# Nazukixv/LiteASR

Hardware: AMD Instinct MI355X
Metric: utterances/sec (U2-Conformer+CTC, 80-d fbank T≈1000) at 1/2/4/8 MI355X (higher is better)
Workload: dtype bf16; 1 GPU; U2-Conformer-small hybrid CTC-attention training step (fwd+loss+bwd+allreduce+clip+Noam/Adam); model=U2 enc 12x conformer d256 H4 ff2048, dec 6x, V 4233, global_batch=32, per_gpu_batch=32, seq_len=1000, label_len=40, parallelism=dp1, launch=hipgraph, ranks_seen=1, rank_launcher=env

## Files before the change

### include/liteasr_hip.h

```cpp
#ifndef LITEASR_HIP_H
#define LITEASR_HIP_H

#include <stdint.h>

#ifdef __cplusplus
extern "C" {
#endif

enum { LASR_F32 = 0, LASR_BF16 = 1, LASR_I32 = 2, LASR_I64 = 3, LASR_U8 = 4 };
enum { LASR_OK = 0, LASR_ERR_INVALID = -1, LASR_ERR_LAUNCH = -2 };
enum { LASR_ACT_NONE = 0, LASR_ACT_RELU = 1, LASR_ACT_SWISH = 2,
       LASR_ACT_GATE = 3 ,
       LASR_ACT_TANH = 4  };

const char* lasr_last_error(void);
int lasr_version(void);
int lasr_set_dropout_counter(const uint64_t* dev_counter);
int lasr_counter_add(uint64_t* dev_counter, uint64_t v, void* stream);

typedef struct lasr_gemm_args {
  int M, N, K;
  int batch, batch_div;
  const void* A; int64_t lda_m, lda_k, sa1, sa2;
  const void* B; int64_t ldb_n, ldb_k, sb1, sb2;
// ... 13 lines not shown
  float* rowsum;
  int zout_mode;
  int tile_m, tile_n;
  int ksub;
} lasr_gemm_args;
int lasr_gemm(const lasr_gemm_args* args, void* stream);
int lasr_gemm_ln_fwd(const lasr_gemm_args* args, const float* gamma, const float* beta, float eps, void* y,
                     int y_dtype, float* mean, float* rstd, void* stream);
int lasr_gemm_ln_bwd(const lasr_gemm_args* args, const void* x, int x_dtype, const float* gamma, const float* mean,
                     const float* rstd, const void* dres, int dres_dtype, void* dx, int dx_dtype, float* part,
                     int64_t part_floats, void* gb, int gb_dtype, float bscale, float bp, uint64_t bseed,
                     void* stream);
int lasr_gemm_qbias_bwd(const lasr_gemm_args* args, const void* dqu, const void* dqv, int dt, int B, int T, int H,
                        int dk, void* dqkv, int64_t ld, float* ws, int64_t ws_floats, void* stream);
float lasr_dropout_scale(float p);
#define LASR_PLAN_GLDS 1
#define LASR_PLAN_ROWSUM_FUSED 2
#define LASR_PLAN_KSUB2 4
#define LASR_PLAN_WIDE 8
int lasr_gemm_plan(const lasr_gemm_args* args, int* tile_m, int* tile_n, int* split_k, int* flags);

int lasr_gemm_dw_group(const lasr_gemm_args* args, int n, void* stream);
int lasr_gemm_dw_group_order(int longest_first);
int lasr_gemm_narrow_tiles(int on);
int lasr_gemm_phased(int mode);
long long lasr_gemm_phased_launches(void);

typedef struct lasr_reduce_seg {
  const float* part; int64_t N; int P; int accumulate;
  float* out0; float* out1; int64_t split;
} lasr_reduce_seg;
int lasr_reduce_multi(const lasr_reduce_seg* segs, int nseg, void* stream);

int lasr_colsum(const void* X, int dtype, int64_t M, int64_t N, int64_t ldx,
                float* out, int accumulate, float* workspace, int64_t ws_floats, void* stream);

int lasr_layernorm_fwd(const void* x, int x_dtype, int64_t rows, int D, const float* gamma,
                       const float* beta, float eps, void* y, int y_dtype, float* mean,
                       float* rstd, void* y2, int y2_dtype, float p2, uint64_t seed2,
                       void* stream);
int lasr_layernorm2_fwd(const float* x, int64_t rows, int D, const float* g1, const float* b1,
                        const float* g2, const float* b2, float eps, float* y, float* mean1,
                        float* rstd1, void* z, float* mean2, float* rstd2, void* stream);
int lasr_layernorm_bwd(const void* x, int x_dtype, const void* dy, int dy_dtype, int64_t rows,
                       int D, const float* gamma, const float* mean, const float* rstd,
                       const void* dres, int dres_dtype, void* dx, int dx_dtype,
// ... 318 lines not shown
```

### liteasr_amd/_native.py

```python

from __future__ import annotations

import ctypes as C
import os

_HERE = os.path.dirname(os.path.abspath(__file__))
LIB_PATH = os.path.join(_HERE, "lib", "libliteasr_hip.so")

F32, BF16, I32, I64, U8 = 0, 1, 2, 3, 4
ACT_NONE, ACT_RELU, ACT_SWISH, ACT_GATE, ACT_TANH = 0, 1, 2, 3, 4

_p = C.c_void_p
_i = C.c_int
_l = C.c_int64
_f = C.c_float
_u = C.c_uint64


class GemmArgs(C.Structure):

    _fields_ = [
        ("M", _i), ("N", _i), ("K", _i),
        ("batch", _i), ("batch_div", _i),
        ("A", _p), ("lda_m", _l), ("lda_k", _l), ("sa1", _l), ("sa2", _l),
# ... 78 lines not shown
class RnntSearchArgs(C.Structure):

    _fields_ = [
        ("Tcap", _i), ("layers", _i), ("dec_dim", _i), ("H", _i), ("J", _i), ("V", _i),
        ("node_cap", _i), ("slot_cap", _i),
        ("w_dtype", _i),
        ("arena", _p), ("arena_bytes", _l),
        ("embed", _p),
        ("Wih", _p * RNNT_SEARCH_MAX_LAYERS), ("Whh", _p * RNNT_SEARCH_MAX_LAYERS),
        ("bih", _p * RNNT_SEARCH_MAX_LAYERS), ("bhh", _p * RNNT_SEARCH_MAX_LAYERS),
        ("Wd", _p), ("Wj", _p), ("bj", _p), ("enc_proj", _p),
    ]


SIGNATURES = {
    "lasr_version": [],
    "lasr_last_error": [],
    "lasr_set_dropout_counter": [_p],
    "lasr_counter_add": [_p, _u, _p],
    "lasr_gemm": [C.POINTER(GemmArgs), _p],
    "lasr_gemm_plan": [C.POINTER(GemmArgs), _p, _p, _p, _p],
    "lasr_gemm_dw_group": [C.POINTER(GemmArgs), _i, _p],
    "lasr_gemm_dw_group_order": [_i],
    "lasr_gemm_narrow_tiles": [_i],
    "lasr_gemm_phased": [_i],
    "lasr_gemm_phased_launches": [],
    "lasr_relattn_fwd": [_p, _p, _l, _p, _p, _l, _p, _l, _i, _i, _i, _i, _p, _l, _l, _f, _p, _p, _l, _p],
    "lasr_relattn_fwd_qb": [_p, _l, _p, _p, _p, _p, _l, _p, _p, _l, _p, _l, _i, _i, _i, _i, _p, _l, _l, _f, _p, _p,
                            _l, _p],
    "lasr_attn_fwd": [_p, _l, _p, _p, _l, _i, _i, _i, _i, _i, _p, _l, _l, _f, _p, _p, _l, _p],
    "lasr_attn_bwd": [_p, _l, _p, _p, _l, _i, _i, _i, _i, _i, _p, _l, _l, _f, _p, _p, _p, _l, _p, _p, _p, _p,
                      _l, _p],
    "lasr_attn_fwd_split": [_p, _l, _p, _p, _l, _i, _i, _i, _i, _i, _p, _l, _l, _f, _p, _p, _l, _i, _p, _l, _p],
    "lasr_attn_bwd_split": [_p, _l, _p, _p, _l, _i, _i, _i, _i, _i, _p, _l, _l, _f, _p, _p, _p, _l, _p, _p, _p,
                            _p, _l, _i, _p, _l, _p],
    "lasr_attn_split_work": [_i, _i, _i, _i, _i],
    "lasr_attn_split_count": [_i, _i, _i, _i],
    "lasr_relattn_bwd": [_p, _p, _l, _p, _p, _l, _p, _l, _i, _i, _i, _i, _p, _l, _l, _f, _p, _p, _p, _l,
                         _p, _p, _p, _i, _i, _p, _p, _l, _p],
    "lasr_reduce_multi": [C.POINTER(ReduceSeg), _i, _p],
    "lasr_linear_res_ln": [C.POINTER(RowLnArgs), _p],
    "lasr_linear_dx_ln_bwd": [C.POINTER(RowLnArgs), _p],
    "lasr_dropout_scale": [_f],
    "lasr_colsum": [_p, _i, _l, _l, _l, _p, _i, _p, _l, _p],
    "lasr_layernorm2_fwd": [_p, _l, _i, _p, _p, _p, _p, _f, _p, _p, _p, _p, _p, _p, _p],
    "lasr_layernorm_fwd": [_p, _i, _l, _i, _p, _p, _f, _p, _i, _p, _p, _p, _i, _f, _u, _p],
# ... 77 lines not shown
    "lasr_rescore_pick_batch": [_p, _l, _i, _i, _i, _p, C.c_double, _p],
    "lasr_w2v_conv0_fwd": [_p, _i, _i, _i, _i, _i, _p, _p, _p, _p],
    "lasr_w2v_conv0_dw_parts": [_i, _i],
    "lasr_w2v_conv0_dw": [_p, _p, _i, _i, _i, _i, _i, _i, _p, _p, _l, _p],
    "lasr_w2v_ln_act_fwd": [_p, _i, _l, _i, _p, _p, _f, _i, _p, _i, _p, _p, _p],
    "lasr_w2v_ln_act_bwd": [_p, _i, _p, _i, _l, _i, _p, _p, _p, _p, _i, _p, _i, _p, _p, _p, _l, _p],
    "lasr_w2v_col2im1d": [_p, _i, _i, _i, _i, _i, _i, _i, _p, _p],
    "lasr_w2v_group_pack": [_p, _i, _i, _i, _i, _i, _i, _p, _i, _p, _p, _i, _p],
    "lasr_w2v_group_unpack": [_p, _i, _p, _i, _p, _i, _i, _i, _i, _p, _p],
    "lasr_w2v_group_colsum": [_p, _i, _i, _l, _i, _p, _p],
    "lasr_w2v_mask_fwd": [_p, _p, _i, _i, _i, _i, _p, _p],
    "lasr_w2v_mask_bwd": [_p, _p, _i, _i, _i, _i, _p, _p],
    "lasr_w2v_gather_rows": [_p, _i, _l, _l, _p, _i, _i, _i, _i, _p, _i, _p],
    "lasr_w2v_scatter_rows": [_p, _i, _p, _i, _i, _i, _i, _p, _l, _l, _i, _p],
    "lasr_w2v_gumbel_fwd": [_p, _i, _p, _u, _f, _i, _l, _i, _i, _p, _i, _p, _i, _p, _p],
    "lasr_w2v_gumbel_bwd": [_p, _i, _p, _u, _f, _i, _l, _i, _i, _p, _i, _p, _i, _p, _p, _i, _p, _p],
    "lasr_w2v_contrast_fwd": [_p, _p, _p, _p, _i, _i, _i, _i, _i, _f, _p, _p, _p, _p, _p],
    "lasr_w2v_contrast_bwd": [_p, _p, _p, _p, _i, _i, _i, _i, _i, _f, _p, _p, _p, _p, _p, _l, _p],
}
_RESTYPES = {"lasr_last_error": C.c_char_p, "lasr_spec_augment_ws_bytes": C.c_int64,
             "lasr_rnnt_search_workspace": C.c_int64, "lasr_rescore_workspace": C.c_int64,
             "lasr_rescore_workspace_batch": C.c_int64, "lasr_ctc_align_workspace": C.c_int64,
             "lasr_conv2_dx_w1_workspace": C.c_int64, "lasr_attn_split_work": C.c_int64,
             "lasr_dropout_scale": C.c_float, "lasr_gemm_phased_launches": C.c_int64}


class NativeError(RuntimeError):
    pass


_lib = None


def load():
    global _lib
    if _lib is not None:
        return _lib
    want = os.environ.get("LITEASR_HIP_LIB")
    if want and os.path.abspath(want) != os.path.abspath(LIB_PATH):
        raise NativeError(f"LITEASR_HIP_LIB={want} does not select the library (this process loads {LIB_PATH}); "
                          "run `python tools/with_lib.py LIB script.py` to use another build")
    if not os.path.exists(LIB_PATH):
        raise NativeError(
            f"libliteasr_hip.so not found at {LIB_PATH}; build it with `make` "
            "(the HIP path has no fallback)"
        )
    lib = C.CDLL(LIB_PATH)
# ... 20 lines not shown
```

### liteasr_amd/csrc/gemm.hip

```cpp
#include "gemm_kernel.h"
#include "gemm_phase.h"
#include <algorithm>


template <bool AKC, bool BKC, typename TC>
void launch_bf16(const GemmP& p, int BM, int BN, int ks, int nw, bool glds, dim3 grid, hipStream_t st);
#define LASR_EXTERN_LAUNCH(ak, bk)                                                                         \
  extern template void launch_bf16<ak, bk, float>(const GemmP&, int, int, int, int, bool, dim3, hipStream_t); \
  extern template void launch_bf16<ak, bk, bf16_t>(const GemmP&, int, int, int, int, bool, dim3, hipStream_t);
LASR_EXTERN_LAUNCH(true, true)
LASR_EXTERN_LAUNCH(true, false)
LASR_EXTERN_LAUNCH(false, true)
LASR_EXTERN_LAUNCH(false, false)
#undef LASR_EXTERN_LAUNCH

template <typename TC>
static void dispatch(const GemmP& p, bool akc, bool bkc, int bf16in, int BM, int BN, int ks, int nw, bool glds,
                     dim3 grid, hipStream_t st) {
  if (bf16in) {
    if (akc && bkc) launch_bf16<true, true, TC>(p, BM, BN, ks, nw, glds, grid, st);
    else if (akc) launch_bf16<true, false, TC>(p, BM, BN, ks, nw, glds, grid, st);
    else if (bkc) launch_bf16<false, true, TC>(p, BM, BN, ks, nw, glds, grid, st);
    else launch_bf16<false, false, TC>(p, BM, BN, ks, nw, glds, grid, st);
  } else {
    if (akc && bkc) gemm_f32_kernel<true, true, TC><<<grid, 256, 0, st>>>(p);
// ... 204 lines not shown
    const int r = post->launch(p, post->ctx, st);
    if (r < 0) return r;
    post->done = r;
    if (r) {
      rc = lasr_check_launch("lasr_gemm/splitk_reduce_post");
      if (rc || !a->rowsum || rs_fused) return rc;
    }
  }
  if (!rc && split > 1 && a->split_k >= 0 && !(post && post->done)) {
    const int64_t total = (int64_t)a->M * a->N * batch;
    const int nblk = (int)std::min<int64_t>(cdiv(p.v4 ? total / 4 : total, 256), 4096);
    if (a->c_dtype == LASR_F32) splitk_reduce_kernel<float><<<nblk, 256, 0, st>>>(p);
    else splitk_reduce_kernel<bf16_t><<<nblk, 256, 0, st>>>(p);
    rc = lasr_check_launch("lasr_gemm/splitk_reduce");
  }
  if (rc || !a->rowsum || rs_fused) return rc;
  const int64_t used = split > 1 ? (int64_t)split * batch * a->M * a->N : 0;
  LASR_CHECK_ARG(a->workspace && a->workspace_bytes / 4 > used, "lasr_gemm: no workspace left for the rowsum");
  return lasr_colsum(a->A, a->in_dtype, a->K, a->M, a->lda_k, a->rowsum, 1, (float*)a->workspace + used,
                     a->workspace_bytes / 4 - used, stream);
}


int launch_dw_group(const DwGroupP& g, int BM, int BN, int blocks, bool serial, hipStream_t st);
static int dw_group_lpt = 1;
extern "C" int lasr_gemm_dw_group_order(int longest_first) {
  dw_group_lpt = longest_first != 0;
  return LASR_OK;
}

extern "C" int lasr_gemm_dw_group(const lasr_gemm_args* args, int n, void* stream) {
  LASR_CHECK_ARG(args && n >= 1 && n <= LASR_DW_GROUP_MAX, "lasr_gemm_dw_group: 1..%d problems", LASR_DW_GROUP_MAX);
  DwGroupP g = {};
  g.n = n;
  int ord[LASR_DW_GROUP_MAX];
  int64_t work[LASR_DW_GROUP_MAX];
  auto planned = [](const lasr_gemm_args* a) {
    lasr_gemm_args b = *a;
    if (b.split_k <= -2 && !b.workspace) {
      b.workspace = (void*)(uintptr_t)16;
      b.workspace_bytes = INT64_MAX;
    }
    return b;
  };
  for (int i = 0; i < n; ++i) {
    const lasr_gemm_args pa = planned(args + i), *a = &pa;
    int bm, bn, sp, ks;
    gemm_plan(a, &bm, &bn, &sp, &ks);
    work[i] = a->split_k == 1 || sp <= 1 ? a->K : cdiv(a->K, sp);
    ord[i] = i;
  }
  if (dw_group_lpt && !(args[0].split_k <= -2 && !args[0].workspace))
    std::stable_sort(ord, ord + n, [&](int x, int y) { return work[x] > work[y]; });
  int BM0 = 0, BN0 = 0, blocks = 0;
  bool all_serial = false;
  for (int i = 0; i < n; ++i) {
    const bool serial = args[ord[i]].split_k <= -2 && !args[ord[i]].workspace;
    const lasr_gemm_args pa = planned(args + ord[i]), *a = &pa;
    LASR_CHECK_ARG(a->in_dtype == LASR_BF16 && a->c_dtype == LASR_F32, "lasr_gemm_dw_group: bf16 in, fp32 partials");
    LASR_CHECK_ARG(a->lda_m == 1 && a->lda_k != 1 && a->ldb_n == 1 && a->ldb_k != 1,
                   "lasr_gemm_dw_group: A M-contiguous and B N-contiguous (dW = dY^T X)");
    const bool direct = a->split_k == 1;
    LASR_CHECK_ARG((direct || (a->split_k < 0 && a->workspace)) && (a->batch <= 1) && a->M > 0 && a->N > 0 &&
                       a->K > 0,
                   "lasr_gemm_dw_group: partials-only problems with a workspace, or direct (split_k 1) ones");
    LASR_CHECK_ARG(!serial || (a->C && a->ldc >= a->N && (a->beta == 0.f || a->beta == 1.f) && a->alpha == 1.f &&
                               !a->alpha_dev && a->split_k >= -64),
                   "lasr_gemm_dw_group: a serial problem needs C, ldc >= N, beta 0 or 1, alpha 1, <= 64 slices");
    LASR_CHECK_ARG(i == 0 || serial == all_serial, "lasr_gemm_dw_group: serial and slab problems mixed");
    all_serial = serial;
    LASR_CHECK_ARG(!direct || (a->C && a->ldc >= a->N && (a->beta == 0.f || a->beta == 1.f) && a->alpha == 1.f &&
                               !a->alpha_dev),
                   "lasr_gemm_dw_group: a direct problem needs C, ldc >= N, beta 0 or 1, alpha 1");
    LASR_CHECK_ARG(i == 0 || direct == (g.direct[0] != 0), "lasr_gemm_dw_group: direct and split problems mixed");
    LASR_CHECK_ARG(!a->act && !a->zout && !a->aux && !a->res && a->drop_p <= 0.f && !a->bias,
                   "lasr_gemm_dw_group: no epilogue");
    LASR_CHECK_ARG(gemm_uses_glds(a), "lasr_gemm_dw_group: operands not LDS-DMA eligible");
    int BM, BN, split, ks;
    gemm_plan(a, &BM, &BN, &split, &ks);
    if (direct) split = 2;
    LASR_CHECK_ARG(split > 1, "lasr_gemm_dw_group: plan is not a split-K launch");
    if (((BM == 128 && BN == 64) || (BM == 64 && BN == 128)) && a->M >= 128 && a->N >= 128) {
      BM = BN = 128;
      if (a->M >= 256 && a->N >= 256 && !direct) {
        BM = 256;
        BN = 128;
      }
    }
    LASR_CHECK_ARG(i == 0 || (BM == BM0 && BN == BN0), "lasr_gemm_dw_group: problems plan different tiles");
    BM0 = BM;
    BN0 = BN;
    if (direct) split = 1;
    g.M[i] = a->M; g.N[i] = a->N; g.K[i] = a->K;
    g.split[i] = split;
    g.kchunk[i] = direct ? a->K : (int)(cdiv(cdiv(a->K, split), 32) * 32);
    g.direct[i] = direct;
    g.C[i] = (float*)a->C; g.ldc[i] = a->ldc; g.beta[i] = a->beta; g.rowsum[i] = a->rowsum;
    g.v4[i] = serial ? a->N % 4 == 0 && aligned16(a->C) && a->ldc % 4 == 0
                     : a->N % 4 == 0 && aligned16(direct ? a->C : a->workspace);
    g.A[i] = a->A; g.lda[i] = a->lda_k;
    g.B[i] = a->B; g.ldb[i] = a->ldb_k;
    g.ws[i] = serial ? nullptr : (float*)a->workspace;
    g.rs_ws[i] = a->rowsum && !direct && !serial ? (float*)a->workspace + (int64_t)split * a->M * a->N : nullptr;
    g.start[i] = blocks;
    const int64_t nb = cdiv(a->M, BM) * cdiv(a->N, BN) * (int64_t)(serial ? 1 : split);
    LASR_CHECK_ARG(blocks + nb + 8 < (1ll << 31), "lasr_gemm_dw_group: too many blocks");
    blocks += (int)cdiv(nb, 8) * 8;
  }
  g.start[n] = blocks;
  static const int slice_xcd = [] { const char* e = getenv("LASR_DW_SLICE_XCD"); return e && e[0] ? atoi(e) : 1; }();
  g.slice_xcd = slice_xcd;
  LASR_CHECK_ARG(launch_dw_group(g, BM0, BN0, blocks, all_serial, (hipStream_t)stream) == 0,
                 "lasr_gemm_dw_group: no grouped instance for tile %dx%d", BM0, BN0);
  return lasr_check_launch("lasr_gemm_dw_group");
}
```

### liteasr_amd/csrc/gemm_group.hip

```cpp
#include "gemm_kernel.h"

static_assert(sizeof(DwGroupP) <= 4096, "DwGroupP must fit the kernel-argument block");

int launch_dw_group(const DwGroupP& g, int BM, int BN, int blocks, bool serial, hipStream_t st) {
  if (serial) {
    if (BM == 64 && BN == 64) gemm_dw_group_kernel<64, 64, 3, 3, 4, true><<<blocks, 256, 0, st>>>(g);
    else if (BM == 256 && BN == 128) gemm_dw_group_kernel<256, 128, 3, 1, 8, true><<<blocks, 512, 0, st>>>(g);
    else return -1;
    return 0;
  }
  if (BM == 64 && BN == 64) gemm_dw_group_kernel<64, 64, 3, 3><<<blocks, 256, 0, st>>>(g);
  else if (BM == 64 && BN == 128) gemm_dw_group_kernel<64, 128, 3, 2><<<blocks, 256, 0, st>>>(g);
  else if (BM == 128 && BN == 64) gemm_dw_group_kernel<128, 64, 3, 2><<<blocks, 256, 0, st>>>(g);
  else if (BM == 128 && BN == 128) gemm_dw_group_kernel<128, 128, 2, 2><<<blocks, 256, 0, st>>>(g);
  else if (BM == 256 && BN == 128) gemm_dw_group_kernel<256, 128, 3, 1, 8><<<blocks, 512, 0, st>>>(g);
  else return -1;
  return 0;
}
```

### liteasr_amd/csrc/gemm_kernel.h

```cpp
#pragma once
#include "common.h"
#include "tile.h"

#include <cstring>
#include <type_traits>

#ifndef LASR_EXP
#define LASR_EXP 0
#endif


struct ConvG {
  int B, T1, F1, T2, F2, C;
  int M2;
  int cls;
  int q32, r32;
  const bf16_t* zero;
  const float* x;
  int T0, F0;
  float* w1part;
  int w1rb;
};
typedef ConvG ConvGeom;
enum { G_LIN = 0, G_FWD = 1, G_DW = 2, G_DX = 3 };
// ... 743 lines not shown
  }
  LASR_DEV void issue(const ConvG& g, const bf16_t* base, bf16_t* dst, int tid) {
    const int wid = tid >> 6;
    const int last = ((g.B * g.T1 - g.T1 + 2 * (g.T2 - 1)) * g.F1 + 2 * (g.F2 - 1)) * g.C;
#pragma unroll
    for (int i = 0; i < PER; ++i) {
      const int rb = b[i] < g.B ? ((b[i] * g.T1 + 2 * t2[i]) * g.F1 + 2 * f2[i]) * g.C : last;
      __builtin_amdgcn_global_load_lds((gptr_t)(base + rb + noff[i]), (lptr_t)(dst + (i * NT + wid * 64) * 8),
                                       16, 0, 0);
      f2[i] += g.r32;
      t2[i] += g.q32;
      if (f2[i] >= g.F2) { f2[i] -= g.F2; t2[i] += 1; }
      while (t2[i] >= g.T2) { t2[i] -= g.T2; b[i] += 1; }
    }
  }
};

LASR_DEV int xcd_remap(int orig, int nwg) {
  const int xcd = orig & 7, q8 = nwg >> 3, r8 = nwg & 7;
  return (xcd < r8 ? xcd * (q8 + 1) : r8 * (q8 + 1) + (xcd - r8) * q8) + (orig >> 3);
}

template <int BM, int BN, bool AKC, bool BKC, typename TC, int S, int G, int KS, int NW = 4, int EPI = EPI_RT,
          bool SERIAL = false>
LASR_DEV void gemm_glds_tile(const GemmP& p, const int tx, const int ty, const int zz) {
  static_assert(G == G_LIN || (G == G_DW ? (!AKC && !BKC) : (AKC && (G == G_FWD) == BKC)),
                "gather instance operand orientation");
  static_assert(!SERIAL || (G == G_LIN && !AKC && !BKC && std::is_same<TC, float>::value && EPI == EPI_RT),
                "serial slices: fp32 weight gradients only");
  static_assert(KS == 1 || KS == 2, "k sub-tiles per ring stage");
  static_assert(NW == 4 || NW == 8, "4 waves (2 x 2) or 8 waves (2 x 4)");
  constexpr int BK = 32;
  constexpr int NT = NW * 64, WCOLS = NW / 2;
  constexpr int WM = BM / 2, WN = BN / WCOLS, FM = WM / 16, FN = WN / 16;
  constexpr int TILE = (BM + BN) * BK;
  constexpr int STAGE = KS * TILE;
  constexpr int MAIN_BYTES = S * STAGE * 2;
  constexpr int EPI_BYTES = WM * (BN + 4) * 4;
  constexpr int GL = (BM + BN) * 4 / NT;
  __shared__ __attribute__((aligned(16))) char smem_epi[MAIN_BYTES > EPI_BYTES ? MAIN_BYTES : EPI_BYTES];
  bf16_t* smem = reinterpret_cast<bf16_t*>(smem_epi);
  const int tid = threadIdx.x, lane = tid & 63, wid = tid >> 6;
  const int wr = wid / WCOLS, wc = wid % WCOLS;

  int s = SERIAL ? 0 : zz % p.split_k;
  const int z = SERIAL ? 0 : zz / p.split_k;
  const int z1 = z / p.batch_div, z2 = z % p.batch_div;
  const bf16_t* A = (const bf16_t*)p.A + z1 * p.sa1 + z2 * p.sa2;
  const bf16_t* B = (const bf16_t*)p.B + z1 * p.sb1 + z2 * p.sb2;
  const int m0 = ty * BM, n0 = tx * BN;
  int kbeg = s * p.kchunk;
  int kend = min(p.K, kbeg + p.kchunk);
  int nk = kend > kbeg ? (kend - kbeg + BK - 1) / BK : 0;
  const int64_t lda = AKC ? p.lda_m : p.lda_k, ldb = BKC ? p.ldb_n : p.ldb_k;

  f32x4 acc[FM][FN];
#pragma unroll
  for (int i = 0; i < FM; ++i)
#pragma unroll
    for (int j = 0; j < FN; ++j) acc[i][j] = (f32x4){0.f, 0.f, 0.f, 0.f};
// ... 77 lines not shown
    if constexpr (!AKC) {
      tie_lgkm<2 * FM>(ra);
#pragma unroll
      for (int i = 0; i < FM; ++i) af[i] = frag_from_raw(ra + 2 * i);
    }
    if constexpr (!BKC) {
      tie_lgkm<2 * FN>(rb);
#pragma unroll
      for (int j = 0; j < FN; ++j) bfr[j] = frag_from_raw(rb + 2 * j);
    }
    if (LASR_EXP & 1) {
#pragma unroll
      for (int i = 0; i < FM; ++i) acc[i][0][0] += (float)af[i][0] + (float)bfr[0][i & 1];
      return;
    }
#pragma unroll
    for (int i = 0; i < FM; ++i)
#pragma unroll
      for (int j = 0; j < FN; ++j)
        acc[i][j] = __builtin_amdgcn_mfma_f32_16x16x32_bf16(bfr[j], af[i], acc[i][j], 0, 0, 0);
  };

  const bool do_rs = !AKC && p.rowsum != nullptr && tx == 0;
  float rs[8];
#pragma unroll
  for (int q = 0; q < 8; ++q) rs[q] = 0.f;

  [[maybe_unused]] f32x4 tot[SERIAL ? FM : 1][SERIAL ? FN : 1];
  [[maybe_unused]] float rs_tot = 0.f;
  if constexpr (SERIAL)
#pragma unroll
    for (int i = 0; i < FM; ++i)
#pragma unroll
      for (int j = 0; j < FN; ++j) tot[i][j] = (f32x4){0.f, 0.f, 0.f, 0.f};
  [[maybe_unused]] int sl = 0;
  do {
    if constexpr (SERIAL) {
      s = sl;
      kbeg = s * p.kchunk;
      kend = min(p.K, kbeg + p.kchunk);
      nk = kend > kbeg ? (kend - kbeg + BK - 1) / BK : 0;
      nfull = (kend - kbeg) > 0 ? (kend - kbeg) / BK : 0;
#pragma unroll
      for (int i = 0; i < FM; ++i)
#pragma unroll
        for (int j = 0; j < FN; ++j) acc[i][j] = (f32x4){0.f, 0.f, 0.f, 0.f};
#pragma unroll
      for (int q = 0; q < 8; ++q) rs[q] = 0.f;
    }
    const int nst = nfull / KS;
#pragma unroll
    for (int t = 0; t < S - 1; ++t)
      if (t < nst) issue(t);

    for (int kt = 0; kt < nst; ++kt) {
      const int after = min(S - 2, nst - 1 - kt);
      wait_ring<S, GL * KS>(after);
      lds_barrier();
      if (kt + S - 1 < nst) issue(kt + S - 1);
#pragma unroll
      for (int u = 0; u < KS; ++u) compute(smem + (kt % S) * STAGE + u * TILE);
      if constexpr (!AKC)
        if (do_rs)
#pragma unroll
          for (int u = 0; u < KS; ++u) rowsum_tile<BM, NT>(smem + (kt % S) * STAGE + u * TILE, tid, rs);
    }
    if constexpr (KS > 1) {
      for (int j = nst * KS; j < nfull; ++j) {
        __syncthreads();
        issue_sub(kbeg + j * BK, smem);
        wait_vmcnt<0>();
        lds_barrier();
        compute(smem);
        if constexpr (!AKC)
          if (do_rs) rowsum_tile<BM, NT>(smem, tid, rs);
      }
    }
    if (G == G_LIN && nfull < nk) {
      __syncthreads();
      TileLoader<BM, AKC, NT> la;
      TileLoader<BN, BKC, NT> lb;
      const int k0 = kbeg + nfull * BK;
      la.load(A, AKC ? p.lda_m : 0, AKC ? 0 : p.lda_k, m0, p.M, k0, kend, true, tid);
      lb.load(B, BKC ? p.ldb_n : 0, BKC ? 0 : p.ldb_k, n0, p.N, k0, kend, true, tid);
      la.store(smem, tid);
      lb.store(smem + BM * BK, tid);
      __syncthreads();
      compute(smem);
      if constexpr (!AKC)
        if (do_rs) rowsum_tile<BM, NT>(smem, tid, rs);
    }
    __syncthreads();
    if constexpr (!AKC) {
      if (do_rs) {
        constexpr int CH = BM / 8, KG = NT / CH;
        float* red = reinterpret_cast<float*>(smem_epi);
        const int c = tid % CH, kg = tid / CH;
#pragma unroll
        for (int q = 0; q < 8; ++q) red[kg * BM + 8 * c + q] = rs[q];
        __syncthreads();
        if (tid < BM) {
          float t = 0.f;
          for (int g = 0; g < KG; ++g) t += red[g * BM + tid];
          const int m = m0 + tid;
          if constexpr (SERIAL) {
            rs_tot += t;
          } else if (m < p.M) {
            if (p.split_k > 1) p.rs_ws[(int64_t)s * p.M + m] = t;
            else p.rowsum[m] += t;
          }
        }
        __syncthreads();
      }
    }
    if constexpr (SERIAL)
#pragma unroll
      for (int i = 0; i < FM; ++i)
#pragma unroll
        for (int j = 0; j < FN; ++j) tot[i][j] += acc[i][j];
  } while (SERIAL && ++sl < p.split_k);
  if constexpr (SERIAL) {
    if (do_rs && tid < BM && m0 + tid < p.M) p.rowsum[m0 + tid] += rs_tot;
    gemm_epilogue_serial<BM, BN, NW>(p, tot, m0, n0);
    return;
  }
  if constexpr (W1) {
// ... 18 lines not shown
  dw_tile_order(wg, nx, ny, !AKC && !BKC && G == G_LIN && p.N > p.M, tx, ty);
  gemm_glds_tile<BM, BN, AKC, BKC, TC, S, G, KS, NW, EPI>(p, tx, ty, blockIdx.z);
}

#define LASR_DW_GROUP_MAX 32
struct DwGroupP {
  int n;
  int start[LASR_DW_GROUP_MAX + 1];
  int M[LASR_DW_GROUP_MAX], N[LASR_DW_GROUP_MAX], K[LASR_DW_GROUP_MAX];
  int split[LASR_DW_GROUP_MAX], kchunk[LASR_DW_GROUP_MAX], v4[LASR_DW_GROUP_MAX];
  const void* A[LASR_DW_GROUP_MAX];
  const void* B[LASR_DW_GROUP_MAX];
  int64_t lda[LASR_DW_GROUP_MAX], ldb[LASR_DW_GROUP_MAX];
  float* ws[LASR_DW_GROUP_MAX];
  float* rs_ws[LASR_DW_GROUP_MAX];
  int slice_xcd;
  int direct[LASR_DW_GROUP_MAX];
  float* C[LASR_DW_GROUP_MAX];
  int64_t ldc[LASR_DW_GROUP_MAX];
  float beta[LASR_DW_GROUP_MAX];
  float* rowsum[LASR_DW_GROUP_MAX];
};

template <int BM, int BN, int S, int MINB, int NW = 4, bool SERIAL = false>
__global__ __launch_bounds__(NW * 64, MINB * NW / 4) void gemm_dw_group_kernel(DwGroupP g) {
  const int blk = blockIdx.x;
  int i = 0;
  for (int j = 1; j < g.n; ++j)
    if (blk >= g.start[j]) i = j;
  const int ntx = (g.N[i] + BN - 1) / BN, nty = (g.M[i] + BM - 1) / BM, ntile = ntx * nty;
  const int local = blk - g.start[i];
  if (local >= (SERIAL ? ntile : ntile * g.split[i])) return;
  GemmP p = {};
  p.M = g.M[i]; p.N = g.N[i]; p.K = g.K[i]; p.batch = 1; p.batch_div = 1;
  p.A = g.A[i]; p.lda_m = 1; p.lda_k = g.lda[i];
  p.B = g.B[i]; p.ldb_n = 1; p.ldb_k = g.ldb[i];
  p.split_k = g.split[i]; p.kchunk = g.kchunk[i]; p.ws = g.ws[i]; p.v4 = g.v4[i];
  p.rowsum = g.rs_ws[i];
  p.rs_ws = g.rs_ws[i];
  p.alpha = 1.f;
  if (g.direct[i]) {
    p.C = g.C[i]; p.ldc = g.ldc[i]; p.beta = g.beta[i];
    p.rowsum = g.rowsum[i]; p.rs_ws = nullptr; p.ws = nullptr;
    p.c_vec = ((uintptr_t)p.C & 15) == 0 && p.ldc % 8 == 0;
    p.epi_mode = p.c_vec && p.beta == 0.f ? 0 : 2;
  }
  if constexpr (SERIAL) {
    p.C = g.C[i]; p.ldc = g.ldc[i]; p.beta = g.beta[i];
    p.rowsum = g.rowsum[i]; p.rs_ws = nullptr; p.ws = nullptr;
    int tx, ty;
    dw_tile_order(xcd_remap(local, ntile), ntx, nty, p.N > p.M, tx, ty);
    gemm_glds_tile<BM, BN, false, false, float, S, G_LIN, 2, NW, EPI_RT, true>(p, tx, ty, 0);
    return;
  }
  int tile, slice;
  const int sp = g.split[i], per = 8 / (sp > 0 ? sp : 1);
  if (g.slice_xcd && 8 % sp == 0 && ntile % per == 0 && (ntile * sp) % 8 == 0) {
    const int x = local & 7, q = local >> 3, run = ntile / per;
    slice = x / per;
    tile = (x % per) * run + q;
  } else {
    tile = xcd_remap(local % ntile, ntile);
    slice = local / ntile;
  }
  int tx, ty;
  dw_tile_order(tile, ntx, nty, p.N > p.M, tx, ty);
  gemm_glds_tile<BM, BN, false, false, float, S, G_LIN, 2, NW>(p, tx, ty, slice);
}

template <bool AKC, bool BKC, typename TC>
__global__ __launch_bounds__(256) void gemm_f32_kernel(GemmP p) {
  constexpr int BM = 64, BN = 64, BK = 16, LD = BK + 1;
  __shared__ float As[BM * LD], Bs[BN * LD];
  const int tid = threadIdx.x, lane = tid & 63, wid = tid >> 6;
  const int wr = wid >> 1, wc = wid & 1;
  const int zz = blockIdx.z;
  const int s = zz % p.split_k, z = zz / p.split_k;
  const int z1 = z / p.batch_div, z2 = z % p.batch_div;
  const float* A = (const float*)p.A + z1 * p.sa1 + z2 * p.sa2;
  const float* B = (const float*)p.B + z1 * p.sb1 + z2 * p.sb2;
  const int m0 = blockIdx.y * BM, n0 = blockIdx.x * BN;
  const int kbeg = s * p.kchunk;
  const int kend = min(p.K, kbeg + p.kchunk);

  f32x4 acc[2][2];
#pragma unroll
  for (int i = 0; i < 2; ++i)
#pragma unroll
    for (int j = 0; j < 2; ++j) acc[i][j] = (f32x4){0.f, 0.f, 0.f, 0.f};

// ... 132 lines not shown
```

### liteasr_amd/csrc/tile.h

```cpp
#pragma once
#include "common.h"

typedef __bf16 bf16x8 __attribute__((ext_vector_type(8)));
typedef float f32x4 __attribute__((ext_vector_type(4)));

LASR_DEV int swz(int row) { return (0x1320 >> (((row >> 2) & 3) * 4)) & 3; }
LASR_DEV int lds_off(int row, int chunk) { return row * 32 + ((chunk ^ swz(row)) << 3); }

LASR_DEV uint4 load8(const bf16_t* src, int start, int lim, bool vec) {
  uint4 v = make_uint4(0, 0, 0, 0);
  if (vec && start + 8 <= lim) {
    v = *(const uint4*)src;
  } else {
    uint32_t e[8];
#pragma unroll
    for (int j = 0; j < 8; ++j) e[j] = (start + j < lim) ? (uint32_t)src[j] : 0u;
    v.x = e[0] | (e[1] << 16);
    v.y = e[2] | (e[3] << 16);
    v.z = e[4] | (e[5] << 16);
    v.w = e[6] | (e[7] << 16);
  }
  return v;
}

// ... 113 lines not shown
  o[0] = 2u * (uint32_t)tr_off<R_TILE>(8 * g + q, rbase + pc);
  o[1] = 2u * (uint32_t)tr_off<R_TILE>(8 * g + 4 + q, rbase + pc);
}
LASR_DEV uint32_t lds_addr(const bf16_t* p) {
  return __builtin_amdgcn_readfirstlane((uint32_t)(uintptr_t)(lptr_t)p);
}
LASR_DEV void frag_tr_raw_at(uint32_t tile_base, const uint32_t* o, v2i* r) {
  asm volatile("ds_read_b64_tr_b16 %0, %1" : "=v"(r[0]) : "v"(tile_base + o[0]));
  asm volatile("ds_read_b64_tr_b16 %0, %1" : "=v"(r[1]) : "v"(tile_base + o[1]));
}
template <int R_TILE>
LASR_DEV void frag_tr_raw(const bf16_t* tile, int rbase, int lane, v2i* r) {
  const int g = lane >> 4, q = (lane >> 2) & 3, pc = (lane & 3) * 4;
  r[0] = ds_tr_asm(tile + tr_off<R_TILE>(8 * g + q, rbase + pc));
  r[1] = ds_tr_asm(tile + tr_off<R_TILE>(8 * g + 4 + q, rbase + pc));
}
typedef int v4i __attribute__((ext_vector_type(4)));
LASR_DEV v4i ds_b128_asm(const bf16_t* p) {
  v4i r;
  const uint32_t a = (uint32_t)(uintptr_t)(lptr_t)p;
  asm volatile("ds_read_b128 %0, %1" : "=v"(r) : "v"(a));
  return r;
}
template <int BM, int NT = 256>
LASR_DEV void rowsum_tile(const bf16_t* tile, int tid, float* rs) {
  constexpr int CH = BM / 8, KG = NT / CH, KR = 32 / KG;
  static_assert(KR >= 1 && KR <= 4 && KR * KG == 32, "rowsum_tile geometry");
  const int c = tid % CH, k0 = tid / CH;
  v4i r[KR];
#pragma unroll
  for (int j = 0; j < KR; ++j) r[j] = ds_b128_asm(tile + tr_off<BM>(k0 + j * KG, 8 * c));
  if constexpr (KR == 1) asm volatile("s_waitcnt lgkmcnt(0)" : "+v"(r[0]));
  else if constexpr (KR == 2) asm volatile("s_waitcnt lgkmcnt(0)" : "+v"(r[0]), "+v"(r[1]));
  else asm volatile("s_waitcnt lgkmcnt(0)" : "+v"(r[0]), "+v"(r[1]), "+v"(r[2]), "+v"(r[3]));
#pragma unroll
  for (int j = 0; j < KR; ++j)
#pragma unroll
    for (int q = 0; q < 4; ++q) {
      const uint32_t u = (uint32_t)r[j][q];
      rs[2 * q] += __uint_as_float(u << 16);
      rs[2 * q + 1] += __uint_as_float(u & 0xffff0000u);
    }
}

LASR_DEV void ds_w64_asm(bf16_t* p, v2i v) {
  const uint32_t a = (uint32_t)(uintptr_t)(lptr_t)p;
  asm volatile("ds_write_b64 %0, %1" ::"v"(a), "v"(v) : "memory");
}
LASR_DEV v2i ds_r64_asm(const bf16_t* p) {
  v2i r;
  const uint32_t a = (uint32_t)(uintptr_t)(lptr_t)p;
  asm volatile("ds_read_b64 %0, %1" : "=v"(r) : "v"(a));
  return r;
}
LASR_DEV v2i pack4_bf16(const float* v) {
  v2i r;
  r[0] = (int)pk_bf16(v[0], v[1]);
  r[1] = (int)pk_bf16(v[2], v[3]);
  return r;
}

LASR_DEV bf16x8 frag_from_raw(const v2i* r) {
  const int __attribute__((ext_vector_type(4))) v = {r[0][0], r[0][1], r[1][0], r[1][1]};
  return __builtin_bit_cast(bf16x8, v);
// ... 28 lines not shown
```

### liteasr_amd/kernels.py

```python

from __future__ import annotations

import contextlib
import os
import ctypes as C
import math
from types import SimpleNamespace
from typing import NamedTuple, Optional

import torch

from . import _native as N

_DT = {torch.float32: N.F32, torch.bfloat16: N.BF16}


def dt(t: torch.Tensor) -> int:
    try:
        return _DT[t.dtype]
    except KeyError:
        raise TypeError(f"unsupported dtype {t.dtype}") from None


def ptr(t: Optional[torch.Tensor]):
# ... 11 lines not shown
        self.frozen = False

    def get(self, nfloats: int, device) -> torch.Tensor:
        nfloats = max(int(nfloats), 1)
        key = torch.device(device).index
        b = self.buf.get(key)
        if b is None or b.numel() < nfloats:
            if self.frozen or torch.cuda.is_current_stream_capturing():
                raise RuntimeError(
                    "workspace growth during graph capture; run a warm-up step first"
                )
            b = torch.empty(int(nfloats * 1.25) + 1024, dtype=torch.float32, device=device)
            self.buf[key] = b
        return b


WS = _Workspace()


DW_GROUP = True
_GROUP_TILES = {(64, 64): (64, 64), (64, 128): (128, 128), (128, 64): (128, 128)}
_GROUP_MAX = 32
DW_GROUP_SPLIT_DIV = {(64, 64): 4, (128, 128): 2}
DW_DIRECT_MIN_TILES = 0
DW_GROUP_LPT = True
DW_HOLD_GEMMS = True
DW_SERIAL_MIN_TILES = 256
DW_HOLD_LAYERS = 4


class Seg(NamedTuple):

    part: torch.Tensor
    P: int
    ncols: int
    out0: torch.Tensor
    out1: Optional[torch.Tensor]
    split: int
    accumulate: int

    @classmethod
    def of(cls, part, P, ncols, out0, out1=None, split=None, accumulate=True):
        return cls(part, int(P), int(ncols), out0, out1, int(ncols if split is None else split), int(accumulate))


class Refs(NamedTuple):
# ... 13 lines not shown

DIRECT_FAMILY = "direct"


def _group_div(key):
    d = DW_GROUP_SPLIT_DIV
    return max(1, d.get(key, 1) if isinstance(d, dict) else int(d))


def _serial_tiles(key, M, Nn):
    if key == (64, 64):
        return -(-M // 64) * -(-Nn // 64)
    if M >= 256 and Nn >= 256:
        return -(-M // 256) * -(-Nn // 128)
    return -(-M // 128) * -(-Nn // 128)


def _dw_slab(sp, M, Nn, rowsum, device):
    nrs = (sp + 128) * M if rowsum is not None else 0
    return torch.empty(sp * M * Nn + nrs, dtype=torch.float32, device=device)


_PUSHED = {}


def _pushed(setter, value):
    if _PUSHED.get(setter) != value:
        N.call(setter, int(value))
        _PUSHED[setter] = value


def _launch_dw_groups(q, before_family=None):
    _pushed("lasr_gemm_dw_group_order", DW_GROUP_LPT)
    families = {}
    for g in q:
        families.setdefault(g.key, []).append(g)
    for key, fam in families.items():
        chunks = [fam[i:i + _GROUP_MAX] for i in range(0, len(fam), _GROUP_MAX)]
        if before_family is not None:
            before_family(key, fam, chunks)
        for ch in chunks:
            arr = (N.GemmArgs * len(ch))(*[g.args for g in ch])
            N.call("lasr_gemm_dw_group", arr, len(ch), stream())


def _reduce(segs):
    arr = (N.ReduceSeg * len(segs))()
    for i, s in enumerate(segs):
        arr[i] = N.ReduceSeg(ptr(s.part), s.ncols, s.P, s.accumulate, ptr(s.out0), ptr(s.out1), s.split)
    N.call("lasr_reduce_multi", arr, len(segs), stream())


def _flush_node_end(segs):
    if _DEFER.gemms:
        _DEFER.flush_gemms()
    if segs:
# ... 1412 lines not shown
```

Measured before the change: 3503 utterances/sec.

## Route large split-K 64x64 weight-grad problems to 256x128 tiles in grouped dW GEMM

In the grouped weight-gradient GEMM, problems that would plan 64x64 tiles with split-K and long K slices are promoted to 256x128 tiles. Serial-mode groups get a persistent scratch slab plus a separate reduce pass. A new RS32 kernel variant keeps per-k rowsum accumulators so the larger 512-thread tile can still fuse the bias rowsum. The aim is better operand reuse and fewer tiny tiles for the big dW GEMMs, at the cost of extra kernel launches, scratch memory, a split reduce and more register pressure.

Result: no change. 3532 utterances/sec, median of 6 (+0.8%).

```diff
diff --git a/include/liteasr_hip.h b/include/liteasr_hip.h
--- a/include/liteasr_hip.h
+++ b/include/liteasr_hip.h
@@ -59,6 +59,9 @@
 
 int lasr_gemm_dw_group(const lasr_gemm_args* args, int n, void* stream);
 int lasr_gemm_dw_group_order(int longest_first);
+#define LASR_DW_DSIZED_MIN_SLICE 1024
+int lasr_gemm_dw_group_dsized(int on, int min_slice);
+long long lasr_gemm_dw_group_dsized_problems(void);
 int lasr_gemm_narrow_tiles(int on);
 int lasr_gemm_phased(int mode);
 long long lasr_gemm_phased_launches(void);
diff --git a/liteasr_amd/_native.py b/liteasr_amd/_native.py
--- a/liteasr_amd/_native.py
+++ b/liteasr_amd/_native.py
@@ -124,6 +124,8 @@
     "lasr_gemm_plan": [C.POINTER(GemmArgs), _p, _p, _p, _p],
     "lasr_gemm_dw_group": [C.POINTER(GemmArgs), _i, _p],
     "lasr_gemm_dw_group_order": [_i],
+    "lasr_gemm_dw_group_dsized": [_i, _i],
+    "lasr_gemm_dw_group_dsized_problems": [],
     "lasr_gemm_narrow_tiles": [_i],
     "lasr_gemm_phased": [_i],
     "lasr_gemm_phased_launches": [],
@@ -247,7 +249,8 @@
              "lasr_rnnt_search_workspace": C.c_int64, "lasr_rescore_workspace": C.c_int64,
              "lasr_rescore_workspace_batch": C.c_int64, "lasr_ctc_align_workspace": C.c_int64,
              "lasr_conv2_dx_w1_workspace": C.c_int64, "lasr_attn_split_work": C.c_int64,
-             "lasr_dropout_scale": C.c_float, "lasr_gemm_phased_launches": C.c_int64}
+             "lasr_dropout_scale": C.c_float, "lasr_gemm_phased_launches": C.c_int64,
+             "lasr_gemm_dw_group_dsized_problems": C.c_int64}
 
 
 class NativeError(RuntimeError):
diff --git a/liteasr_amd/csrc/gemm.hip b/liteasr_amd/csrc/gemm.hip
--- a/liteasr_amd/csrc/gemm.hip
+++ b/liteasr_amd/csrc/gemm.hip
@@ -1,6 +1,8 @@
 #include "gemm_kernel.h"
 #include "gemm_phase.h"
 #include <algorithm>
+#include <atomic>
+#include <mutex>
 
 
 template <bool AKC, bool BKC, typename TC>
@@ -251,27 +253,115 @@
 }
 
 
-int launch_dw_group(const DwGroupP& g, int BM, int BN, int blocks, bool serial, hipStream_t st);
+int launch_dw_group(const DwGroupP& g, int BM, int BN, int blocks, bool serial, bool rs32, hipStream_t st);
 static int dw_group_lpt = 1;
 extern "C" int lasr_gemm_dw_group_order(int longest_first) {
   dw_group_lpt = longest_first != 0;
   return LASR_OK;
 }
+static int dw_group_dsized = 1, dw_group_dsized_min_slice = LASR_DW_DSIZED_MIN_SLICE;
+extern "C" int lasr_gemm_dw_group_dsized(int on, int min_slice) {
+  LASR_CHECK_ARG(min_slice >= 0, "lasr_gemm_dw_group_dsized: min_slice >= 0");
+  dw_group_dsized = on != 0;
+  dw_group_dsized_min_slice = min_slice;
+  return LASR_OK;
+}
+static std::atomic<long long> dw_dsized_count{0};
+extern "C" long long lasr_gemm_dw_group_dsized_problems(void) { return dw_dsized_count.load(std::memory_order_relaxed); }
+
+static lasr_gemm_args dw_planned(const lasr_gemm_args* a) {
+  lasr_gemm_args b = *a;
+  if (b.split_k <= -2 && !b.workspace) {
+    b.workspace = (void*)(uintptr_t)16;
+    b.workspace_bytes = INT64_MAX;
+  }
+  return b;
+}
+
+static int dw_dsized_split(const lasr_gemm_args* a0) {
+  if (!dw_group_dsized || a0->split_k >= 0 || a0->in_dtype != LASR_BF16 || a0->M < 256 || a0->N < 256 || a0->K <= 0)
+    return 0;
+  const lasr_gemm_args a = dw_planned(a0);
+  int bm, bn, sp, ks;
+  gemm_plan(&a, &bm, &bn, &sp, &ks);
+  return bm == 64 && bn == 64 && sp > 1 && cdiv(a.K, sp) >= dw_group_dsized_min_slice ? sp : 0;
+}
+
+static float* dw_dsized_scratch(int64_t bytes, hipStream_t st) {
+  static std::mutex mu;
+  static struct { float* p; int64_t cap; } cur[64] = {};
+  int dev = 0;
+  if (hipGetDevice(&dev) != hipSuccess || dev < 0 || dev >= 64) return nullptr;
+  std::lock_guard<std::mutex> lock(mu);
+  if (cur[dev].cap >= bytes) return cur[dev].p;
+  hipStreamCaptureStatus cs = hipStreamCaptureStatusNone;
+  if (hipStreamIsCapturing(st, &cs) != hipSuccess || cs != hipStreamCaptureStatusNone) {
+    (void)hipGetLastError();
+    return nullptr;
+  }
+  void* p = nullptr;
+  const int64_t cap = bytes + bytes / 4;
+  if (hipMalloc(&p, (size_t)cap) != hipSuccess) {
+    (void)hipGetLastError();
+    return nullptr;
+  }
+  cur[dev].p = (float*)p;
+  cur[dev].cap = cap;
+  return cur[dev].p;
+}
+
+static int dw_group_launch(const lasr_gemm_args* args, int n, void* stream);
 
 extern "C" int lasr_gemm_dw_group(const lasr_gemm_args* args, int n, void* stream) {
   LASR_CHECK_ARG(args && n >= 1 && n <= LASR_DW_GROUP_MAX, "lasr_gemm_dw_group: 1..%d problems", LASR_DW_GROUP_MAX);
+  const bool serial = args[0].split_k <= -2 && !args[0].workspace;
+  lasr_gemm_args E[LASR_DW_GROUP_MAX], R[LASR_DW_GROUP_MAX];
+  int sp[LASR_DW_GROUP_MAX], ne = 0, nr = 0;
+  int64_t need = 0;
+  for (int i = 0; i < n; ++i) {
+    const int s = (args[i].split_k <= -2 && !args[i].workspace) == serial ? dw_dsized_split(args + i) : 0;
+    if (s && (!serial || (args[i].C && ((int64_t)args[i].M * args[i].N) % 4 == 0 && args[i].ldc == args[i].N &&
+                          (!args[i].rowsum || args[i].M % 4 == 0)))) {
+      sp[ne] = s;
+      E[ne++] = args[i];
+      need += ((int64_t)s * args[i].M * args[i].N + (args[i].rowsum ? (int64_t)s * args[i].M : 0) + 3) / 4 * 4;
+    } else {
+      R[nr++] = args[i];
+    }
+  }
+  if (ne == 0) return dw_group_launch(args, n, stream);
+  if (!serial) {
+    int rc = dw_group_launch(E, ne, stream);
+    if (!rc && nr) rc = dw_group_launch(R, nr, stream);
+    if (!rc) dw_dsized_count += ne;
+    return rc;
+  }
+  float* ws = dw_dsized_scratch(need * 4, (hipStream_t)stream);
+  if (!ws) return dw_group_launch(args, n, stream);
+  lasr_reduce_seg segs[2 * LASR_DW_GROUP_MAX];
+  int ns = 0;
+  for (int i = 0; i < ne; ++i) {
+    lasr_gemm_args& a = E[i];
+    const int64_t mn = (int64_t)a.M * a.N, fl = (int64_t)sp[i] * mn + (a.rowsum ? (int64_t)sp[i] * a.M : 0);
+    a.workspace = ws;
+    a.workspace_bytes = fl * 4;
+    segs[ns++] = lasr_reduce_seg{ws, mn, sp[i], a.beta == 1.f, (float*)a.C, nullptr, mn};
+    if (a.rowsum) segs[ns++] = lasr_reduce_seg{ws + (int64_t)sp[i] * mn, a.M, sp[i], 1, a.rowsum, nullptr, a.M};
+    ws += (fl + 3) / 4 * 4;
+  }
+  int rc = dw_group_launch(E, ne, stream);
+  if (!rc) rc = lasr_reduce_multi(segs, ns, stream);
+  if (!rc && nr) rc = dw_group_launch(R, nr, stream);
+  if (!rc) dw_dsized_count += ne;
+  return rc;
+}
+
+static int dw_group_launch(const lasr_gemm_args* args, int n, void* stream) {
   DwGroupP g = {};
   g.n = n;
   int ord[LASR_DW_GROUP_MAX];
   int64_t work[LASR_DW_GROUP_MAX];
-  auto planned = [](const lasr_gemm_args* a) {
-    lasr_gemm_args b = *a;
-    if (b.split_k <= -2 && !b.workspace) {
-      b.workspace = (void*)(uintptr_t)16;
-      b.workspace_bytes = INT64_MAX;
-    }
-    return b;
-  };
+  auto planned = [](const lasr_gemm_args* a) { return dw_planned(a); };
   for (int i = 0; i < n; ++i) {
     const lasr_gemm_args pa = planned(args + i), *a = &pa;
     int bm, bn, sp, ks;
@@ -282,7 +372,7 @@
   if (dw_group_lpt && !(args[0].split_k <= -2 && !args[0].workspace))
     std::stable_sort(ord, ord + n, [&](int x, int y) { return work[x] > work[y]; });
   int BM0 = 0, BN0 = 0, blocks = 0;
-  bool all_serial = false;
+  bool all_serial = false, rs32_0 = false;
   for (int i = 0; i < n; ++i) {
     const bool serial = args[ord[i]].split_k <= -2 && !args[ord[i]].workspace;
     const lasr_gemm_args pa = planned(args + ord[i]), *a = &pa;
@@ -316,9 +406,16 @@
         BN = 128;
       }
     }
-    LASR_CHECK_ARG(i == 0 || (BM == BM0 && BN == BN0), "lasr_gemm_dw_group: problems plan different tiles");
+    const bool rs32 = BM == 64 && BN == 64 && !direct && !serial && dw_dsized_split(args + ord[i]) > 0;
+    if (rs32) {
+      BM = 256;
+      BN = 128;
+    }
+    LASR_CHECK_ARG(i == 0 || (BM == BM0 && BN == BN0 && rs32 == rs32_0),
+                   "lasr_gemm_dw_group: problems plan different tiles");
     BM0 = BM;
     BN0 = BN;
+    rs32_0 = rs32;
     if (direct) split = 1;
     g.M[i] = a->M; g.N[i] = a->N; g.K[i] = a->K;
     g.split[i] = split;
@@ -339,7 +436,7 @@
   g.start[n] = blocks;
   static const int slice_xcd = [] { const char* e = getenv("LASR_DW_SLICE_XCD"); return e && e[0] ? atoi(e) : 1; }();
   g.slice_xcd = slice_xcd;
-  LASR_CHECK_ARG(launch_dw_group(g, BM0, BN0, blocks, all_serial, (hipStream_t)stream) == 0,
+  LASR_CHECK_ARG(launch_dw_group(g, BM0, BN0, blocks, all_serial, rs32_0, (hipStream_t)stream) == 0,
                  "lasr_gemm_dw_group: no grouped instance for tile %dx%d", BM0, BN0);
   return lasr_check_launch("lasr_gemm_dw_group");
 }
diff --git a/liteasr_amd/csrc/gemm_group.hip b/liteasr_amd/csrc/gemm_group.hip
--- a/liteasr_amd/csrc/gemm_group.hip
+++ b/liteasr_amd/csrc/gemm_group.hip
@@ -2,7 +2,13 @@
 
 static_assert(sizeof(DwGroupP) <= 4096, "DwGroupP must fit the kernel-argument block");
 
-int launch_dw_group(const DwGroupP& g, int BM, int BN, int blocks, bool serial, hipStream_t st) {
+int launch_dw_group(const DwGroupP& g, int BM, int BN, int blocks, bool serial, bool rs32, hipStream_t st) {
+  if (rs32) {
+    if (serial) return -1;
+    if (BM == 256 && BN == 128) gemm_dw_group_kernel<256, 128, 3, 1, 8, false, true><<<blocks, 512, 0, st>>>(g);
+    else return -1;
+    return 0;
+  }
   if (serial) {
     if (BM == 64 && BN == 64) gemm_dw_group_kernel<64, 64, 3, 3, 4, true><<<blocks, 256, 0, st>>>(g);
     else if (BM == 256 && BN == 128) gemm_dw_group_kernel<256, 128, 3, 1, 8, true><<<blocks, 512, 0, st>>>(g);
diff --git a/liteasr_amd/csrc/gemm_kernel.h b/liteasr_amd/csrc/gemm_kernel.h
--- a/liteasr_amd/csrc/gemm_kernel.h
+++ b/liteasr_amd/csrc/gemm_kernel.h
@@ -789,7 +789,7 @@
 }
 
 template <int BM, int BN, bool AKC, bool BKC, typename TC, int S, int G, int KS, int NW = 4, int EPI = EPI_RT,
-          bool SERIAL = false>
+          bool SERIAL = false, bool RS32 = false>
 LASR_DEV void gemm_glds_tile(const GemmP& p, const int tx, const int ty, const int zz) {
   static_assert(G == G_LIN || (G == G_DW ? (!AKC && !BKC) : (AKC && (G == G_FWD) == BKC)),
                 "gather instance operand orientation");
@@ -803,6 +803,8 @@
   constexpr int TILE = (BM + BN) * BK;
   constexpr int STAGE = KS * TILE;
   constexpr int MAIN_BYTES = S * STAGE * 2;
+  constexpr int RSJ = RS32 ? 32 / (NT / (BM / 8)) : 1;
+  static_assert(!RS32 || MAIN_BYTES >= 32 * BM * 4, "RS32 combine slab (32 x BM floats)");
   constexpr int EPI_BYTES = WM * (BN + 4) * 4;
   constexpr int GL = (BM + BN) * 4 / NT;
   __shared__ __attribute__((aligned(16))) char smem_epi[MAIN_BYTES > EPI_BYTES ? MAIN_BYTES : EPI_BYTES];
@@ -926,9 +928,9 @@
   };
 
   const bool do_rs = !AKC && p.rowsum != nullptr && tx == 0;
-  float rs[8];
-#pragma unroll
-  for (int q = 0; q < 8; ++q) rs[q] = 0.f;
+  float rs[8 * RSJ];
+#pragma unroll
+  for (int q = 0; q < 8 * RSJ; ++q) rs[q] = 0.f;
 
   [[maybe_unused]] f32x4 tot[SERIAL ? FM : 1][SERIAL ? FN : 1];
   [[maybe_unused]] float rs_tot = 0.f;
@@ -950,7 +952,7 @@
 #pragma unroll
         for (int j = 0; j < FN; ++j) acc[i][j] = (f32x4){0.f, 0.f, 0.f, 0.f};
 #pragma unroll
-      for (int q = 0; q < 8; ++q) rs[q] = 0.f;
+      for (int q = 0; q < 8 * RSJ; ++q) rs[q] = 0.f;
     }
     const int nst = nfull / KS;
 #pragma unroll
@@ -967,7 +969,7 @@
       if constexpr (!AKC)
         if (do_rs)
 #pragma unroll
-          for (int u = 0; u < KS; ++u) rowsum_tile<BM, NT>(smem + (kt % S) * STAGE + u * TILE, tid, rs);
+          for (int u = 0; u < KS; ++u) rowsum_tile<BM, NT, RS32>(smem + (kt % S) * STAGE + u * TILE, tid, rs);
     }
     if constexpr (KS > 1) {
       for (int j = nst * KS; j < nfull; ++j) {
@@ -977,7 +979,7 @@
         lds_barrier();
         compute(smem);
         if constexpr (!AKC)
-          if (do_rs) rowsum_tile<BM, NT>(smem, tid, rs);
+          if (do_rs) rowsum_tile<BM, NT, RS32>(smem, tid, rs);
       }
     }
     if (G == G_LIN && nfull < nk) {
@@ -992,7 +994,7 @@
       __syncthreads();
       compute(smem);
       if constexpr (!AKC)
-        if (do_rs) rowsum_tile<BM, NT>(smem, tid, rs);
+        if (do_rs) rowsum_tile<BM, NT, RS32>(smem, tid, rs);
     }
     __syncthreads();
     if constexpr (!AKC) {
@@ -1001,11 +1003,13 @@
         float* red = reinterpret_cast<float*>(smem_epi);
         const int c = tid % CH, kg = tid / CH;
 #pragma unroll
-        for (int q = 0; q < 8; ++q) red[kg * BM + 8 * c + q] = rs[q];
+        for (int j = 0; j < RSJ; ++j)
+#pragma unroll
+          for (int q = 0; q < 8; ++q) red[(kg + j * KG) * BM + 8 * c + q] = rs[8 * j + q];
         __syncthreads();
         if (tid < BM) {
           float t = 0.f;
-          for (int g = 0; g < KG; ++g) t += red[g * BM + tid];
+          for (int g = 0; g < KG * RSJ; ++g) t += red[g * BM + tid];
           const int m = m0 + tid;
           if constexpr (SERIAL) {
             rs_tot += t;
@@ -1070,7 +1074,7 @@
   float* rowsum[LASR_DW_GROUP_MAX];
 };
 
-template <int BM, int BN, int S, int MINB, int NW = 4, bool SERIAL = false>
+template <int BM, int BN, int S, int MINB, int NW = 4, bool SERIAL = false, bool RS32 = false>
 __global__ __launch_bounds__(NW * 64, MINB * NW / 4) void gemm_dw_group_kernel(DwGroupP g) {
   const int blk = blockIdx.x;
   int i = 0;
@@ -1113,7 +1117,7 @@
   }
   int tx, ty;
   dw_tile_order(tile, ntx, nty, p.N > p.M, tx, ty);
-  gemm_glds_tile<BM, BN, false, false, float, S, G_LIN, 2, NW>(p, tx, ty, slice);
+  gemm_glds_tile<BM, BN, false, false, float, S, G_LIN, 2, NW, EPI_RT, false, RS32>(p, tx, ty, slice);
 }
 
 template <bool AKC, bool BKC, typename TC>
diff --git a/liteasr_amd/csrc/tile.h b/liteasr_amd/csrc/tile.h
--- a/liteasr_amd/csrc/tile.h
+++ b/liteasr_amd/csrc/tile.h
@@ -159,7 +159,7 @@
   asm volatile("ds_read_b128 %0, %1" : "=v"(r) : "v"(a));
   return r;
 }
-template <int BM, int NT = 256>
+template <int BM, int NT = 256, bool PER_K = false>
 LASR_DEV void rowsum_tile(const bf16_t* tile, int tid, float* rs) {
   constexpr int CH = BM / 8, KG = NT / CH, KR = 32 / KG;
   static_assert(KR >= 1 && KR <= 4 && KR * KG == 32, "rowsum_tile geometry");
@@ -175,8 +175,9 @@
 #pragma unroll
     for (int q = 0; q < 4; ++q) {
       const uint32_t u = (uint32_t)r[j][q];
-      rs[2 * q] += __uint_as_float(u << 16);
-      rs[2 * q + 1] += __uint_as_float(u & 0xffff0000u);
+      float* a = rs + (PER_K ? 8 * j : 0);
+      a[2 * q] += __uint_as_float(u << 16);
+      a[2 * q + 1] += __uint_as_float(u & 0xffff0000u);
     }
 }
 
diff --git a/liteasr_amd/kernels.py b/liteasr_amd/kernels.py
--- a/liteasr_amd/kernels.py
+++ b/liteasr_amd/kernels.py
@@ -57,6 +57,8 @@
 _GROUP_TILES = {(64, 64): (64, 64), (64, 128): (128, 128), (128, 64): (128, 128)}
 _GROUP_MAX = 32
 DW_GROUP_SPLIT_DIV = {(64, 64): 4, (128, 128): 2}
+DW_GROUP_DSIZED = True
+DW_DSIZED_MIN_SLICE = 1024
 DW_DIRECT_MIN_TILES = 0
 DW_GROUP_LPT = True
 DW_HOLD_GEMMS = True
@@ -116,16 +118,18 @@
 
 
 _PUSHED = {}
+_LIB_DEFAULTS = {"lasr_gemm_dw_group_dsized": (DW_GROUP_DSIZED, DW_DSIZED_MIN_SLICE)}
 
 
 def _pushed(setter, value):
-    if _PUSHED.get(setter) != value:
-        N.call(setter, int(value))
+    if _PUSHED.get(setter, _LIB_DEFAULTS.get(setter)) != value:
+        N.call(setter, *(map(int, value) if isinstance(value, tuple) else (int(value),)))
         _PUSHED[setter] = value
 
 
 def _launch_dw_groups(q, before_family=None):
     _pushed("lasr_gemm_dw_group_order", DW_GROUP_LPT)
+    _pushed("lasr_gemm_dw_group_dsized", (bool(DW_GROUP_DSIZED), int(DW_DSIZED_MIN_SLICE)))
     families = {}
     for g in q:
         families.setdefault(g.key, []).append(g)
```
